# Tomeu7/AO-MARL

Hardware: AMD Instinct MI355X
Metric: env steps/sec (AO frames/sec) (higher is better)
Workload: dtype f32

## Files before the change

### __graft_entry__.py

```python
import os
import subprocess
import sys

ROOT = os.path.dirname(os.path.abspath(__file__))
if ROOT not in sys.path:
    sys.path.insert(0, ROOT)


def build():
    subprocess.check_call(["make", "-s", "-C", os.path.join(ROOT, "ao_marl_amd", "csrc")])
    subprocess.check_call(["make", "-s", "-C", os.path.join(ROOT, "oracle")])
    import ao_marl_amd
    from ao_marl_amd import libaomarl
    libaomarl.load()
    from oracle import aoref
    aoref.lib()


def smoke():
    import numpy as np
    import torch
    from ao_marl_amd.sim import HipSim
    from oracle import aoref
    sys.path.insert(0, os.path.join(ROOT, "tests"))
    from tests import helpers
    assert torch.cuda.is_available(), "smoke() needs a GPU"
    _, s, cal = helpers.calibrated("production_sh_10x10_2m")
    seeds = [1234, 1250]
    sim = HipSim(s, nenv=len(seeds))
    sim.set_modal(cal.volts2modes, cal.modes2volts)
    sim.reset(seeds)
    oracles = [aoref.OracleSim(s, seed=sd) for sd in seeds]
    for _ in range(2):
        sim.next_part_two(None)
        sim.next_part_one()
        for o in oracles:
            o.next_part_two(None)
            o.next_part_one()
    torch.cuda.synchronize()
    sl = sim.slopes.cpu().numpy()
    cm = sim.com.cpu().numpy()
    st = sim.strehl.cpu().numpy()
    for e, o in enumerate(oracles):
# ... 12 lines not shown
```

### ao_marl_amd/csrc/aomarl_capi.hip

```cpp
#include "aomarl_kernels.hip"

#include <math.h>
#include <stdlib.h>
#include <stdarg.h>
#include <stdio.h>
#include <string.h>

#include <algorithm>
#include <climits>
#include <string>
#include <vector>

static thread_local char g_err[512] = "";

int fail(const char *fmt, ...) {
  va_list ap;
  va_start(ap, fmt);
  vsnprintf(g_err, sizeof(g_err), fmt, ap);
  va_end(ap);
  return 1;
}


struct aomarl_ctx {
// ... 732 lines not shown
static Work work_layout(const aomarl_ctx *c, int nenv) {
  Work w;
  const DevSys &s = c->sys;
  const size_t ncol = (size_t)nenv * (c->nlayers > 0 ? c->nlayers : 1);
  w.ldz = (c->maxK + 3) & ~3;
  w.ldn = (c->maxdim + 3) & ~3;
  w.ldm = (s.nactu + 3) & ~3;
  const int W = 2 * s.hw, RB = 256 / W;
  w.nblk = (s.pupdiam + RB - 1) / RB;
  size_t o = 0;
  auto take = [&](size_t n) { size_t r = o; o += (n + 3) & ~(size_t)3; return r; };
  w.Z = take(ncol * w.ldz);
  w.NEWL = take(ncol * w.ldn);
  w.ZREF = take(ncol);
  w.Z2 = take(ncol * w.ldz);
  w.ZREF2 = take(ncol);
  w.MODES = take((size_t)nenv * w.ldm);
  w.TR = take((size_t)nenv * s.pupdiam * W * 2);
  w.TPART = take((size_t)nenv * w.nblk * 4);
  w.PEND = take((size_t)nenv * (W * W + 4));
  {
    size_t mn = std::max(ncol * (size_t)w.ldn, (size_t)nenv * (size_t)w.ldm);
    w.gemm_floats = 8 * mn;
    w.GEMM = take(w.gemm_floats);
    w.GEMM_ATM = take(w.gemm_floats);
  }
  w.total = o;
  return w;
}

size_t aomarl_workspace_floats(const aomarl_ctx *c, int nenv) {
  return c ? work_layout(c, nenv).total : 0;
}
size_t aomarl_screen_stride(const aomarl_ctx *c) { return c ? (size_t)c->sys.screen_stride : 0; }
size_t aomarl_dmshape_stride(const aomarl_ctx *c) { return c ? (size_t)c->sys.shape_stride : 0; }

static int check_range(const aomarl_ctx *c, const aomarl_state *st, int b, int n) {
  if (!c || !st) return fail("null ctx/state");
  if (c->pipe.active && !c->pipe_internal && st->screens == c->pipe.owner_screens)
    return fail("a pipelined frame is in flight on this state (aomarl_set_frame_pipeline): only aomarl_env_step and a "
                "full-range aomarl_reset are accepted until the reset -- slopes / voltage of odd frames are in the twin, "
                "the screens a frame ahead");
  if (b < 0 || n < 0 || b + n > st->nenv) return fail("env range [%d, %d) outside [0, %d)", b, b + n, st->nenv);
  if (st->ld_actu < c->sys.nactu) return fail("ld_actu (%d) < nactu (%d)", st->ld_actu, c->sys.nactu);
  if (!st->screens || !st->origin || !st->seeds || !st->ext_count || !st->com || !st->com1 ||
      !st->com2 || !st->err || !st->voltage || !st->slopes || !st->dm_shape || !st->strehl ||
      !st->le_img || !st->frame || !st->work)
    return fail("aomarl_state has a null mandatory buffer");
  return 0;
}

static DevState dev_state(const aomarl_state *st) {
  DevState d;
  d.nenv = st->nenv; d.ld_actu = st->ld_actu;
  d.screens = st->screens; d.origin = st->origin; d.seeds = st->seeds; d.ext_count = st->ext_count;
  d.com = st->com; d.com1 = st->com1; d.com2 = st->com2; d.err = st->err; d.voltage = st->voltage;
  d.slopes = st->slopes; d.dm_shape = st->dm_shape; d.bincube = st->bincube;
  d.wfs_phase = st->wfs_phase; d.tar_phase = st->tar_phase; d.strehl = st->strehl;
  d.le_img = st->le_img; d.frame = st->frame; d.work = st->work;
  d.origin_snap = nullptr;
  return d;
}

#include "aomarl_capi_atmos.hip"
#include "aomarl_capi_stages.hip"
#include "aomarl_capi_agents.hip"
// ... 4 lines not shown
```

### ao_marl_amd/csrc/aomarl_capi_composites.hip

```cpp
const char *aomarl_frame_kernel_name(aomarl_ctx *c) {
  if (!c || !c->fw_variant[0]) return "";
  snprintf(c->fw_name, sizeof(c->fw_name), "k_frame_wave<%d, %d, %s, %s, %s, %s>", c->fw_variant[0], c->fw_variant[1],
           c->fw_variant[2] ? "true" : "false", c->fw_variant[3] ? "true" : "false",
           c->fw_variant[4] ? "true" : "false", c->fw_variant[5] ? "true" : "false");
  return c->fw_name;
}

int aomarl_frame_kernel_time(aomarl_ctx *c, double *total_ms, int *launches) {
  if (!c || !total_ms || !launches) return fail("frame_kernel_time: null argument");
  double tot = 0.0;
  int n = 0;
  for (size_t i = 0; i + 1 < c->fw_ev_used; i += 2) {
    float ms = 0.f;
    HIPCHK(hipEventSynchronize(c->fw_ev[i + 1]));
    HIPCHK(hipEventElapsedTime(&ms, c->fw_ev[i], c->fw_ev[i + 1]));
    tot += ms; n++;
  }
  { const int rrc = fw_ev_rewind(c); if (rrc) return rrc; }
  *total_ms = tot; *launches = n;
  return 0;
}

int aomarl_frame_fused_available(aomarl_ctx *c) {
  return c && c->sys.fused_ok && !c->force_unfused_frame ? 1 : 0;
}

static int frame_fused_impl(aomarl_ctx *c, aomarl_state *st, int b, int n, int flags, void *stream, int slot);

int aomarl_frame_fused(aomarl_ctx *c, aomarl_state *st, int b, int n, int flags, void *stream) {
  return frame_fused_impl(c, st, b, n, flags, stream, -1);
}

static int frame_fused_impl(aomarl_ctx *c, aomarl_state *st, int b, int n, int flags, void *stream, int slot) {
  int rc = check_range(c, st, b, n);
  if (rc) return rc;
  if (slot < 0) {
    rc = atmos_wait_pending(c, stream);
    if (rc) return rc;
    rc = psf_wait_pending(c, stream);
    if (rc) return rc;
  }
  if (!c->sys.fused_ok) return fail("frame_fused: geometry not eligible (see aomarl_frame_fused_available)");
  if (flags & (AOMARL_IMG_FROM_PHASE_BUFFER | AOMARL_IMG_NO_ATMOS | AOMARL_IMG_NO_DMS))
    return fail("frame_fused: FROM_PHASE_BUFFER / NO_ATMOS / NO_DMS are not supported here");
  const bool noise = (flags & AOMARL_IMG_NOISE) && c->sys.noise >= 0.f;
  const bool cube = flags & AOMARL_IMG_WRITE_BINCUBE;
  const bool otf = flags & AOMARL_IMG_DM_FROM_VOLTAGE;
  const int cog = ((flags & AOMARL_IMG_COG) ? 1 : 0) | (c->fused_debug << 8);
  if (otf && !c->sys.otf_ok) return fail("frame_fused: DM_FROM_VOLTAGE needs a separable stack-array lattice (see aomarl_dm_from_voltage_available)");
  if (cube && !st->bincube) return fail("frame_fused: WRITE_BINCUBE needs st->bincube");
  if (!cube && !(cog & 1)) return fail("frame_fused: nothing to produce (neither bincube nor slopes)");
  if (n == 0) return 0;
  hipStream_t s = (hipStream_t)stream;
  Work w = work_layout(c, st->nenv);
  const int W = 2 * c->sys.hw;
  float *TR = st->work + w.TR + (size_t)b * c->sys.pupdiam * W * 2;
  float *TP = st->work + w.TPART + (size_t)b * w.nblk * 4;
  float *PEND = st->work + w.PEND + (size_t)b * (W * W + 4);
  DevState ds = dev_state(st);
  if (w.nblk != c->sys.ntiles) return fail("frame_fused: internal stripe count mismatch");
  const int nb = otf ? c->sys.otf_nb : 1;
  const bool hp = c->dft_mode < 0 ? g_precision != 0 : c->dft_mode == 1;
  const bool qf = FW_QF && otf && !hp && !noise && !cube;
  const bool dma = FW_DMA && otf && (hp || FW_DMA_F32);
  const size_t smm = sizeof(float) * ((qf ? 0 : 2 * 128) + (otf ? 4 * 4 * nb * c->sys.otf_latw : 0)) + FW_SLOT_BYTES(dma) +
                     (dma ? 4 * FWD_WAVE(c->nlayers == 1 ? 1 : 3) : 128) +
                     (qf ? 4 * 16 * (size_t)c->sys.ntiles : 0);
  static const long lds_pad_env = [] { const char *e = getenv("AOMARL_FW_LDS_PAD"); return e ? atol(e) : -1L; }();
  size_t lds_pad = 0;
  if (qf && slot >= 0 && smm >= 40 * 1024) {
    const size_t two_per_cu = (160 * 1024) / 3 + 64;
    lds_pad = lds_pad_env >= 0 ? (size_t)lds_pad_env : (smm < two_per_cu ? (two_per_cu - smm + 63) / 64 * 64 : 0);
    if (smm + lds_pad > 64 * 1024) lds_pad = 0;
  }
  dim3 grid((n + 3) / 4, c->sys.ntiles), blk(256);
#define FW(NL, NB, OTF, NZ, WC, HP) hipExtLaunchKernelGGL((k_frame_wave<NL, NB, OTF, NZ, WC, HP>), grid, blk, smm + lds_pad, s, ev_start, ev_done, 0, c->sys, ds, b, n, cog, TR, TP, w.nblk)
#define FW_H(NL, NB, OTF, NZ, WC) do { if (hp) FW(NL, NB, OTF, NZ, WC, true); else FW(NL, NB, OTF, NZ, WC, false); } while (0)
#define FW_NC(NL, NB, OTF)                                                                     \
  do {                                                                                          \
    if (noise) { if (cube) FW_H(NL, NB, OTF, true, true); else FW_H(NL, NB, OTF, true, false); }     \
    else { if (cube) FW_H(NL, NB, OTF, false, true); else FW_H(NL, NB, OTF, false, false); }         \
  } while (0)
#define FW_L(NL)                                                          \
  do {                                                                    \
    if (!otf) FW_NC(NL, 1, false);                                        \
    else if (nb == 1) FW_NC(NL, 1, true);                                 \
    else FW_NC(NL, 2, true);                                              \
  } while (0)
  const bool timed = !c->capturing && c->time_fw && c->fw_ev_used + 2 <= c->fw_ev.size();
  hipEvent_t ev_start = nullptr, ev_done = nullptr;
  if (c->prefetch_atmos) {
    rc = side_stream(c);
    if (rc) return rc;
    ev_done = slot < 0 ? c->ev_frame : c->pipe.ev_done[slot];
  }
  if (timed) { ev_start = c->fw_ev[c->fw_ev_used]; ev_done = c->fw_ev[c->fw_ev_used + 1]; c->fw_ev_used += 2; }
  hipEvent_t ev_mark = nullptr;
  if (c->capturing) { ev_mark = ev_done; ev_start = nullptr; ev_done = nullptr; }
  if (c->nlayers == 1) FW_L(1); else FW_L(3);
  if (ev_mark) { HIPCHK(hipEventRecord(ev_mark, s)); ev_done = ev_mark; }
  c->frame_marked = false;
  c->fw_variant[0] = c->nlayers == 1 ? 1 : 3; c->fw_variant[1] = otf ? nb : 1; c->fw_variant[2] = otf;
  c->fw_variant[3] = noise; c->fw_variant[4] = cube; c->fw_variant[5] = hp;
  g_arith[hp ? AR_FRAME_SPLIT : AR_FRAME_F32]++;
#undef FW_L
#undef FW_NC
#undef FW_H
// ... 189 lines not shown
```

### ao_marl_amd/csrc/aomarl_kernels.hip

```cpp
#include "aomarl_host.h"
#include "aomarl_gemm_p.h"
#include <type_traits>

#define WAVE 64

typedef unsigned u32x4 __attribute__((ext_vector_type(4)));

__device__ __forceinline__ hx2 cvt_h2(float a, float b) {
  return __builtin_bit_cast(hx2, __builtin_amdgcn_cvt_pkrtz(a, b));
}
__device__ __forceinline__ float sub_lo(hx2 h, float a) {
  float r;
  asm("v_fma_mix_f32 %0, %1, -1.0, %2 op_sel_hi:[1,0,0]" : "=v"(r) : "v"(h), "v"(a));
  return r;
}
__device__ __forceinline__ float sub_hi(hx2 h, float a) {
  float r;
  asm("v_fma_mix_f32 %0, %1, -1.0, %2 op_sel:[1,0,0] op_sel_hi:[1,0,0]" : "=v"(r) : "v"(h), "v"(a));
  return r;
}

struct __attribute__((packed, aligned(4))) f4u { float v[4]; };
__device__ __forceinline__ void add4(float acc[4], const float *p) {
  const f4u t = *reinterpret_cast<const f4u *>(p);
// ... 2056 lines not shown

typedef const int __attribute__((address_space(4))) *const_int_p;
typedef const float __attribute__((address_space(4))) *const_float_p;

template <int NL, bool OTF>
struct FrameRaw {
  float L[NL][4];
  float P[OTF ? 1 : 4], T[8];
  unsigned mrow;
  float F;
  f4u SH;
  float4 CS;
};

template <int NL, int NB, bool OTF, bool NOISE, bool WRITE_CUBE, bool HP>
#ifndef FW_WAVES
#define FW_WAVES 3
#endif
#ifndef FW_QF
#define FW_QF 1
#endif
#ifndef FW_DMA
#define FW_DMA 1
#endif
#ifndef FW_DEPTH
#define FW_DEPTH 2
#endif
#ifndef FW_DMA_F32
#define FW_DMA_F32 1
#endif
#ifndef FW_SLOTS1
#define FW_SLOTS1 0
#endif
#define FW_SLOT_BYTES(dma) ((dma) ? (FW_SLOTS1 ? 2 * 3 * 1024 : 16384) : 16384)
#define FWD_BLK 1152
#define FWD_IMG (2 * 1024 + 128)
#define FWD_WAVE(nl) ((nl) * FWD_IMG)
__global__ __launch_bounds__(256) __attribute__((amdgpu_waves_per_eu(FW_WAVES, FW_WAVES)))
void k_frame_wave(DevSys sys, DevState st, int env_begin,
                                                    int env_count, int do_cog,
                                                    float *__restrict__ TR,
                                                    float *__restrict__ TPART, int nblk) {
  extern __shared__ float smem[];
  const int pd = sys.pupdiam, ntl = sys.ntiles;
  const int tid = threadIdx.x, lane = tid & 63, q = lane >> 4, c = lane & 15;
  const int wv = __builtin_amdgcn_readfirstlane(tid >> 6);
  constexpr bool QF = FW_QF && OTF && !HP && !NOISE && !WRITE_CUBE;
  constexpr bool DMA = FW_DMA && OTF && (HP || FW_DMA_F32);
  float2 *sTw = reinterpret_cast<float2 *>(smem);
  float *lat_all = reinterpret_cast<float *>(sTw + (QF ? 0 : 128));
  float4 *shb = reinterpret_cast<float4 *>(lat_all + 4 * 4 * NB * (OTF ? sys.otf_latw : 0));
  char *dimg = reinterpret_cast<char *>(shb) + FW_SLOT_BYTES(DMA) + (DMA ? wv * FWD_WAVE(NL) : 0);
  float4 *qmom = reinterpret_cast<float4 *>(reinterpret_cast<char *>(shb) + FW_SLOT_BYTES(DMA) + (DMA ? 4 * FWD_WAVE(NL) : 0)) + wv * ntl;
  const int dbg = do_cog >> 8;
  do_cog &= 1;
  const int r = sys.stripe_order[blockIdx.y];
  const int el = 4 * blockIdx.x + wv;
  if constexpr (!QF) {
    if (tid < 128) {
      float sn, cs;
      sincospif((float)tid * (1.0f / 64.0f), &sn, &cs);
      sTw[tid] = make_float2(cs, sn);
    }
    __syncthreads();
  }
  const bool active = el < env_count;
  const int e = env_begin + (active ? el : env_count - 1);
// ... 130 lines not shown
  };

  auto tile = [&](int info, int infon, FrameRaw<NL, OTF> &cur, FrameRaw<NL, OTF> &nxt, auto mode_tag, float4 *dma_slot) {
    constexpr bool DM = decltype(mode_tag)::value == 1;
    constexpr bool NOFETCH = decltype(mode_tag)::value != 0;
    const int t = (info >> 24) & 0x7F;
    f32x4 S = PK ? NP4 : Z4;
    if (OTF) {
      f32x4 U = Z4;
#pragma unroll
      for (int kb = 0; kb < NB; kb++) {
        const float a = latq[(q + 4 * kb) * latw + t * tpn];
        U = mfma16(jm_ok ? a : 0.f, Pyr[kb], U);
      }
#pragma unroll
      for (int s = 0; s < NB; s++) S = mfma16(Pxr[s], U[s], S);
    }
    const float flux_i = cur.F;
    float4 *slot = DM ? dma_slot : shb + (nlit & 1) * 256;
    if constexpr (!DM) {
      nlit++;
      slot[wv * 64 + lane] = make_float4(cur.SH.v[0], cur.SH.v[1], cur.SH.v[2], cur.SH.v[3]);
#ifndef FW_DBG_NOBAR
      __syncthreads();
#endif
    }
    if (!(DM && FW_SLOTS1)) {
      const float4 t0 = slot[lane], t1 = slot[64 + lane];
      cur.T[0] = t0.x; cur.T[1] = t0.y; cur.T[2] = t0.z; cur.T[3] = t0.w;
      cur.T[4] = t1.x; cur.T[5] = t1.y; cur.T[6] = t1.z; cur.T[7] = t1.w;
      cur.CS = slot[128 + lane];
    }
    const float4 csP = cur.CS;
    float wr[4], wi[4], ar[4], ai[4];
    if constexpr (PK) {
      const f32x2 X01 = {cur.T[0], cur.T[1]}, X23 = {cur.T[2], cur.T[3]};
      const f32x2 Y01 = {cur.T[4], cur.T[5]}, Y23 = {cur.T[6], cur.T[7]};
      PK_GUARD_MFMA();
      f32x2 p01 = pk_fma_s(X01, c0c0, pk_lo(S)), p23 = pk_fma_s(X23, c0c0, pk_hi(S));
      p01 = pk_fma_s(Y01, c1c1, p01); p23 = pk_fma_s(Y23, c1c1, p23);
#pragma unroll
      for (int l = 0; l < NL; l++) {
        const f32x2 l01 = {cur.L[l][0], cur.L[l][1]}, l23 = {cur.L[l][2], cur.L[l][3]};
        p01 = pk_add(p01, l01); p23 = pk_add(p23, l23);
      }
      if (info & FW_FULL) {
        const f32x2 t01 = pk_mul_s(p01, wil2), t23 = pk_mul_s(p23, wil2);
        const f32x2 b01 = pk_mul_s(p01, til2), b23 = pk_mul_s(p23, til2);
        if constexpr (QF) {
          sdp += p01; sd2p = __builtin_elementwise_fma(p01, p01, sd2p);
          sdp += p23; sd2p = __builtin_elementwise_fma(p23, p23, sd2p);
          wr[0] = __builtin_amdgcn_cosf(t01.x); wi[0] = __builtin_amdgcn_sinf(t01.x);
          wr[1] = __builtin_amdgcn_cosf(t01.y); wi[1] = __builtin_amdgcn_sinf(t01.y);
          wr[2] = __builtin_amdgcn_cosf(t23.x); wi[2] = __builtin_amdgcn_sinf(t23.x);
          wr[3] = __builtin_amdgcn_cosf(t23.y); wi[3] = __builtin_amdgcn_sinf(t23.y);
        } else {
        sdp += p01; sd2p = __builtin_elementwise_fma(p01, p01, sd2p);
        const f32x2 r01 = {rintf(t01.x), rintf(t01.y)}, r23 = {rintf(t23.x), rintf(t23.y)};
        sdp += p23; sd2p = __builtin_elementwise_fma(p23, p23, sd2p);
        const f32x2 a01 = pk_fma_nc_s(p01, wil2, r01), a23 = pk_fma_nc_s(p23, wil2, r23);
        wr[0] = __builtin_amdgcn_cosf(a01.x); wi[0] = __builtin_amdgcn_sinf(a01.x);
        wr[1] = __builtin_amdgcn_cosf(a01.y); wi[1] = __builtin_amdgcn_sinf(a01.y);
        wr[2] = __builtin_amdgcn_cosf(a23.x); wi[2] = __builtin_amdgcn_sinf(a23.x);
        wr[3] = __builtin_amdgcn_cosf(a23.y); wi[3] = __builtin_amdgcn_sinf(a23.y);
        }
        ar[0] = __builtin_amdgcn_cosf(b01.x); ai[0] = __builtin_amdgcn_sinf(b01.x);
        ar[1] = __builtin_amdgcn_cosf(b01.y); ai[1] = __builtin_amdgcn_sinf(b01.y);
        ar[2] = __builtin_amdgcn_cosf(b23.x); ai[2] = __builtin_amdgcn_sinf(b23.x);
        ar[3] = __builtin_amdgcn_cosf(b23.y); ai[3] = __builtin_amdgcn_sinf(b23.y);
        nfull++;
      } else {
        const float ph4[4] = {p01.x, p01.y, p23.x, p23.y};
#pragma unroll
        for (int j = 0; j < 4; j++) {
          const float ph = ph4[j];
          const bool m = (cur.mrow >> (4 * q + j)) & 1u;
          float a_ = ph * wfs_il; a_ -= rintf(a_);
          const float b_ = sci_rev(ph, tar_il);
          wr[j] = m ? __builtin_amdgcn_cosf(a_) : 0.f; wi[j] = m ? __builtin_amdgcn_sinf(a_) : 0.f;
          ar[j] = m ? __builtin_amdgcn_cosf(b_) : 0.f; ai[j] = m ? __builtin_amdgcn_sinf(b_) : 0.f;
          const float d = m ? ph : 0.f;
          sd += d; sd2 += d * d; sm += m ? 1.f : 0.f;
        }
      }
    } else if (info & FW_FULL) {
#pragma unroll
      for (int j = 0; j < 4; j++) {
        float ph = (OTF ? S[j] : cur.P[OTF ? 0 : j]) + (c0 * cur.T[j] + c1 * cur.T[4 + j]);
#pragma unroll
        for (int l = 0; l < NL; l++) ph += cur.L[l][j];
        float a_ = ph * wfs_il; a_ -= rintf(a_);
        const float b_ = sci_rev(ph, tar_il);
        wr[j] = __builtin_amdgcn_cosf(a_); wi[j] = __builtin_amdgcn_sinf(a_);
        ar[j] = __builtin_amdgcn_cosf(b_); ai[j] = __builtin_amdgcn_sinf(b_);
        const float d = ph - pivot;
        sd += d; sd2 += d * d;
      }
      sm += 4.f;
    } else {
#pragma unroll
      for (int j = 0; j < 4; j++) {
        float ph = (OTF ? S[j] : cur.P[OTF ? 0 : j]) + (c0 * cur.T[j] + c1 * cur.T[4 + j]);
#pragma unroll
        for (int l = 0; l < NL; l++) ph += cur.L[l][j];
        const bool m = (cur.mrow >> (4 * q + j)) & 1u;
        float a_ = ph * wfs_il; a_ -= rintf(a_);
        const float b_ = sci_rev(ph, tar_il);
        wr[j] = m ? __builtin_amdgcn_cosf(a_) : 0.f; wi[j] = m ? __builtin_amdgcn_sinf(a_) : 0.f;
        ar[j] = m ? __builtin_amdgcn_cosf(b_) : 0.f; ai[j] = m ? __builtin_amdgcn_sinf(b_) : 0.f;
        const float d = m ? ph - pivot : 0.f;
        sd += d; sd2 += d * d; sm += m ? 1.f : 0.f;
      }
    }
    if constexpr (!NOFETCH) fetch(infon, nxt);
    if (!(dbg & 2)) {
      if constexpr (PK) {
        const f32x2 ar01 = {ar[0], ar[1]}, ar23 = {ar[2], ar[3]}, ai01 = {ai[0], ai[1]}, ai23 = {ai[2], ai[3]};
        PK_GUARD_TRANS();
        const f32x2 sr_ = pk_add(ar01, ar23), si_ = pk_add(ai01, ai23);
        pk_acc_add(R0rp, sr_); pk_acc_add(R0ip, si_);
        PK_END_TO_MFMA();
      } else {
        R0r += (ar[0] + ar[1]) + (ar[2] + ar[3]);
        R0i += (ai[0] + ai[1]) + (ai[2] + ai[3]);
      }
      if (HP) {
        const hx8 csH = __builtin_bit_cast(hx8, csP);
        hx8 arH, arL, aiH, aiL;
        dup_hl(ar[0], ar[1], ar[2], ar[3], arH, arL);
        dup_hl(ai[0], ai[1], ai[2], ai[3], aiH, aiL);
        PA = mfma_h(arH, csH, PA); PA = mfma_h(arL, csH, PA);
        PB = mfma_h(aiH, csH, PB); PB = mfma_h(aiL, csH, PB);
      } else {
        PA = mfma16(ar[0], csP.x, PA); PB = mfma16(ai[0], csP.x, PB);
        PA = mfma16(ar[1], csP.y, PA); PB = mfma16(ai[1], csP.y, PB);
        PA = mfma16(ar[2], csP.z, PA); PB = mfma16(ai[2], csP.z, PB);
        PA = mfma16(ar[3], csP.w, PA); PB = mfma16(ai[3], csP.w, PB);
      }
// ... 7 lines not shown
        if constexpr (QF) {
          const float z = spot_qf_moments(qfk, wr, wi, Z4);
          if (c == 0 && q < 3) reinterpret_cast<float *>(qmom + t)[q] = z;
        } else if constexpr (PK) spot_cog_f32_pk(sys, st, e, info & 0xFFFF, lane, Cc, Ss, wr, wi, do_cog, Z4);
        else spot_cog_f32(sys, st, e, info & 0xFFFF, lane, Cc, Ss, wr, wi, do_cog, Z4);
      } else {
        spot_core<NOISE, WRITE_CUBE>(sys, st, e, info & 0xFFFF, lane, Cc, Ss, wr, wi, do_cog, flux_i, Z4);
      }
    }
  };

  if constexpr (DMA) {
    const std::integral_constant<int, 1> dm;
    const int np = sys.pair_count[r];
    const const_int_p pinfo = (const_int_p)(unsigned long long)(sys.pair_info + r * (2 * ((ntl + 1) / 2 + 2)));
    const int rr = lane >> 3, kk = (lane & 7) ^ rr;
    unsigned dvo[NL][2];
#pragma unroll
    for (int l = 0; l < NL; l++) {
      const DevLayer &L = sys.layers[l];
      int py = L.toy + st.origin[(e * sys.nlayers + l) * 2 + 1]; py -= (py >= L.dim) ? L.dim : 0;
#pragma unroll
      for (int b = 0; b < 2; b++) {
        unsigned pr = (unsigned)(16 * r + 8 * b + rr) + (unsigned)py; pr = min(pr, pr - ldim[l]);
        dvo[l][b] = 4u * (pr * (ldim[l] + RING_PAD)) + 16u * (unsigned)kk;
      }
    }
    const int bc = c >> 3, rc = c & 7;
    const char *rdp[2];
#pragma unroll
    for (int h = 0; h < 2; h++) rdp[h] = dimg + bc * FWD_BLK + 16 * (rc * 8 + ((4 * h + q) ^ rc));
    const unsigned dimg_lds = (unsigned)(unsigned long long)dimg;
    FrameRaw<NL, OTF> A, B;
    unsigned mrA, mrB;
    float fA, fB;
    const unsigned shb_lds = (unsigned)(unsigned long long)shb + 1024u * (unsigned)wv;
    auto dma16 = [&](unsigned vo, __amdgpu_buffer_rsrc_t rs, unsigned lds_addr, unsigned so) {
      unsigned keep;
      asm volatile("s_mov_b32 %0, m0\n\ts_mov_b32 m0, %3\n\ts_nop 0\n\tbuffer_load_dwordx4 %1, %2, %4 offen lds\n\ts_mov_b32 m0, %0"
                   : "=&s"(keep) : "v"(vo), "s"(rs), "s"(lds_addr), "s"(so) : "memory");
    };
    auto issue_shared = [&](int ia, int ib, int par) {
      const int ta = (ia >> 24) & 0x7F, tb = (ib >> 24) & 0x7F;
      if (FW_SLOTS1) {
        if (wv < 3) {
          dma16(shvo, shrs, shb_lds, (unsigned)ta << shstep);
          dma16(shvo, shrs, shb_lds + 3072u, (unsigned)tb << shstep);
        }
      } else {
        dma16(shvo, shrs, shb_lds + (unsigned)par * 8192u, (unsigned)ta << shstep);
        dma16(shvo, shrs, shb_lds + (unsigned)par * 8192u + 4096u, (unsigned)tb << shstep);
      }
    };
    auto issue = [&](int ia, int ib) {
      const int ta = (ia >> 24) & 0x7F, tb = (ib >> 24) & 0x7F;
      mrA = *reinterpret_cast<const uint16_t *>(mkb + 2u * (unsigned)ta + mvo);
      mrB = *reinterpret_cast<const uint16_t *>(mkb + 2u * (unsigned)tb + mvo);
      fA = cflux[ia & 0xFFFF];
      fB = cflux[ib & 0xFFFF];
#pragma unroll
      for (int l = 0; l < NL; l++) {
        unsigned sx = 16u * (unsigned)(ta & ~1) + lpxs[l]; sx -= (sx >= ldim[l]) ? ldim[l] : 0u;
        const unsigned so = 4u * sx;
#pragma unroll
        for (int b = 0; b < 2; b++) dma16(dvo[l][b], lrs[l], dimg_lds + l * FWD_IMG + b * FWD_BLK, so);
      }
    };
    int ia = pinfo[0], ib = pinfo[1];
    if (np > 0) { issue_shared(ia, ib, 0); issue(ia, ib); }
    for (int k = 0; k < np; k++) {
      const int ja = pinfo[2 * k + 2], jb = pinfo[2 * k + 3];
      asm volatile("s_waitcnt vmcnt(0)" ::: "memory");
#pragma unroll
      for (int l = 0; l < NL; l++) {
        const float4 va = *reinterpret_cast<const float4 *>(rdp[0] + l * FWD_IMG);
        const float4 vb = *reinterpret_cast<const float4 *>(rdp[1] + l * FWD_IMG);
        A.L[l][0] = va.x; A.L[l][1] = va.y; A.L[l][2] = va.z; A.L[l][3] = va.w;
        B.L[l][0] = vb.x; B.L[l][1] = vb.y; B.L[l][2] = vb.z; B.L[l][3] = vb.w;
      }
      A.mrow = mrA; A.F = fA; B.mrow = mrB; B.F = fB;
      asm volatile("s_waitcnt lgkmcnt(0)" ::: "memory");
      if (FW_SLOTS1) {
        if (k + 1 < np) issue(ja, jb);
        __syncthreads();
        float4 *slots = shb;
        {
          const float4 a0 = slots[lane], a1 = slots[64 + lane];
          A.CS = slots[128 + lane];
          A.T[0] = a0.x; A.T[1] = a0.y; A.T[2] = a0.z; A.T[3] = a0.w; A.T[4] = a1.x; A.T[5] = a1.y; A.T[6] = a1.z; A.T[7] = a1.w;
        }
        if (ia & FW_LIT) tile(ia, 0, A, A, dm, slots);
        {
          const float4 b0 = slots[192 + lane], b1 = slots[256 + lane];
          B.CS = slots[320 + lane];
          B.T[0] = b0.x; B.T[1] = b0.y; B.T[2] = b0.z; B.T[3] = b0.w; B.T[4] = b1.x; B.T[5] = b1.y; B.T[6] = b1.z; B.T[7] = b1.w;
        }
        asm volatile("s_waitcnt lgkmcnt(0)" ::: "memory");
        __syncthreads();
        if (k + 1 < np) issue_shared(ja, jb, 0);
        if (ib & FW_LIT) tile(ib, 0, B, B, dm, slots);
      } else {
        float4 *slots = shb + (k & 1) * 512;
        __syncthreads();
        if (k + 1 < np) { issue_shared(ja, jb, (k + 1) & 1); issue(ja, jb); }
        if (ia & FW_LIT) tile(ia, 0, A, A, dm, slots);
        if (ib & FW_LIT) tile(ib, 0, B, B, dm, slots + 256);
      }
      ia = ja; ib = jb;
    }
  } else {
  const std::integral_constant<int, 0> nd;
  const std::integral_constant<int, 2> nf;
  const int nl = sys.lit_count[r];
  const const_int_p linfo = (const_int_p)(unsigned long long)(sys.lit_info + r * (ntl + 8));
  {
    constexpr int D = FW_DEPTH;
    FrameRaw<NL, OTF> raw[D];
    int inf[D];
#pragma unroll
    for (int d = 0; d < D; d++) { inf[d] = linfo[d]; fetch(inf[d], raw[d]); }
    const int rem = nl % D, nfull = nl - rem;
    for (int k = 0; k < nfull; k += D) {
      int nx[D];
#pragma unroll
      for (int d = 0; d < D; d++) nx[d] = linfo[k + D + d];
#pragma unroll
      for (int d = 0; d < D; d++) tile(inf[d], nx[d], raw[d], raw[d], nd, nullptr);
#pragma unroll
      for (int d = 0; d < D; d++) inf[d] = nx[d];
    }
#pragma unroll
    for (int d = 0; d + 1 < D; d++)
      if (rem > d) tile(inf[d], inf[d], raw[d], raw[d], nf, nullptr);
  }
  }
  if (!active) return;
  if constexpr (QF) {
    if (do_cog && !(dbg & 1)) {
      for (int tt = lane; tt < ntl; tt += 64) {
// ... 830 lines not shown
```

### ao_marl_amd/libaomarl.py

```python
import ctypes as C
import os
import subprocess

import numpy as np

HERE = os.path.dirname(os.path.abspath(__file__))
LIB_PATH = os.environ.get("AOMARL_LIB") or os.path.join(HERE, "libaomarl_hip.so")
MAX_LAYERS, MAX_DMS, ABI_VERSION = 8, 4, 2
PRECISION_F32, PRECISION_SPLIT_F16 = 0, 1

DM_PZT, DM_TT = 0, 1
TRACE_ATMOS, TRACE_DMS, TRACE_RESET, TRACE_MASK = 1, 2, 4, 8
IMG_FROM_PHASE_BUFFER, IMG_NOISE, IMG_WRITE_BINCUBE, IMG_COG, IMG_NO_ATMOS, IMG_NO_DMS = \
    1, 2, 4, 8, 16, 32
IMG_DM_FROM_VOLTAGE = 64
APPLY_COMP_VOLTAGE, APPLY_DEFER_STACK_SHAPE = 1, 2

_fp = C.POINTER(C.c_float)
_ip = C.POINTER(C.c_int32)
_up = C.POINTER(C.c_uint32)


class DmDesc(C.Structure):
    _fields_ = [("type", C.c_int32), ("dim", C.c_int32), ("nact", C.c_int32),
# ... 107 lines not shown
    ("aomarl_actor_forward", _i, [_vp, _vp, _vp, C.c_uint32, C.c_uint32, _vp, _vp, _vp]),
    ("aomarl_env_step", _i, [_vp, C.POINTER(State), _vp, _vp, _f, _fp, _fp, _vp, _vp, _vp]),
    ("aomarl_policy_env_step", _i, [_vp, C.POINTER(State), _vp, _vp, _vp, _vp, C.c_uint32, C.c_uint32, _f, _fp, _fp,
                                    _vp, _vp, _vp, _vp, _vp]),
    ("aomarl_env_step_shortcut", _i, [_vp, _vp]),
    ("aomarl_do_control_reduced", _i, [_vp, C.POINTER(State), _vp]),
    ("aomarl_graph_stats", _i, [_vp, C.POINTER(C.c_ulonglong), C.POINTER(C.c_ulonglong)]),
    ("aomarl_set_frame_pipeline", _i, [_vp, C.POINTER(State), C.POINTER(State)]),
    ("aomarl_frame_pipeline_state", _i, [_vp, C.POINTER(_i), C.POINTER(_i), C.POINTER(C.c_ulonglong),
                                         C.POINTER(C.c_ulonglong)]),
    ("aomarl_frame_kernel_name", C.c_char_p, [_vp]),
    ("aomarl_frame_kernel_time", _i, [_vp, C.POINTER(C.c_double), C.POINTER(_i)]),
    ("aomarl_denoiser_create", _i, [C.POINTER(_fp), C.POINTER(_fp), C.POINTER(C.c_void_p)]),
    ("aomarl_denoiser_apply", _i, [_vp, _vp, C.c_longlong, _vp]),
    ("aomarl_denoiser_apply_f32", _i, [_vp, _vp, C.c_longlong, _vp]),
    ("aomarl_denoiser_apply_split_f16", _i, [_vp, _vp, C.c_longlong, _vp]),
    ("aomarl_denoiser_overflow", _i, [_vp, C.POINTER(C.c_uint), _vp]),
    ("aomarl_denoiser_destroy", _i, [_vp]),
    ("aomarl_denoiser_trainer_create", _i, [C.POINTER(_fp), C.POINTER(_fp), C.c_double, C.c_double, C.c_double,
                                            C.c_double, _i, C.POINTER(C.c_void_p)]),
    ("aomarl_denoiser_trainer_destroy", _i, [_vp]),
    ("aomarl_denoiser_trainer_step", _i, [_vp, _vp, _vp, C.c_longlong, _vp, _vp]),
    ("aomarl_denoiser_trainer_grads", _i, [_vp, _vp, _vp, C.c_longlong, C.POINTER(C.c_void_p),
                                           C.POINTER(C.c_void_p), _vp, _vp]),
    ("aomarl_denoiser_trainer_get", _i, [_vp, C.POINTER(C.c_void_p), C.POINTER(C.c_void_p), _vp]),
    ("aomarl_target_psf_buffer", _i, _range + [_vp]),
    ("aomarl_set_geo", _i, [_vp, _fp]),
    ("aomarl_geo_workspace_floats", C.c_size_t, [_vp, _i]),
    ("aomarl_geo_control", _i, _range + [_vp, _vp]),
    ("aomarl_frame_fused_available", _i, [_vp]),
    ("aomarl_dm_from_voltage_available", _i, [_vp]),
    ("aomarl_materialize_dm_shape", _i, _range + [_vp]),
    ("aomarl_frame_fused", _i, _range + [_i, _vp]),
    ("aomarl_comp_strehl", _i, _range + [_vp]),
    ("aomarl_reset_strehl", _i, _range + [_vp]),
    ("aomarl_volts2modes", _i, [_vp, C.POINTER(State), _i, _vp, _i, _vp, _vp]),
    ("aomarl_set_slopes2modes", _i, [_vp, _i, _fp]),
    ("aomarl_slopes2modes", _i, _range + [_vp, _vp]),
    ("aomarl_next_part_one", _i, _range + [_fp, _fp, _i, _vp]),
    ("aomarl_next_part_two", _i, _range + [_vp, _vp]),
    ("aomarl_gemm_nt", _i, [_i, _i, _i, _f, _vp, _i, _vp, _i, _f, _vp, _i, _vp]),
    ("aomarl_gemm_nt_split", _i, [_i, _i, _i, _f, _vp, _i, _vp, _i, _f, _vp, _i, _f, _f, _vp, C.c_longlong, _vp]),
    ("aomarl_gemm_nt_batched", _i, [_i, _i, _i, _i, _vp, _i, C.c_longlong, _vp, _i, C.c_longlong,
                                    _vp, C.c_longlong, _vp, _i, C.c_longlong, _i, _vp]),
]

_lib = None


class SacDesc(C.Structure):
    _fields_ = [(n, C.c_int32) for n in ("n_agents", "batch", "in_max", "act_max", "hidden", "hidden_critic",
                                         "n_hidden",
                                         "state_dim", "action_dim")] + \
               [("state_gather", C.c_void_p), ("action_gather", C.c_void_p), ("n_act", C.c_void_p),
                ("target_entropy", C.c_void_p)] + \
               [(n, C.c_float) for n in ("gamma", "tau", "lr", "beta1", "beta2", "adam_eps", "log_sig_min",
                                         "log_sig_max", "action_scale", "action_bias")] + \
               [(n, C.c_void_p) for n in ("policy", "policy_m", "policy_v", "policy_grad", "critic",
                                          "critic_m", "critic_v", "critic_grad", "critic_target",
                                          "log_alpha", "log_alpha_m", "log_alpha_v", "log_alpha_grad",
                                          "alpha")]


class ActorDesc(C.Structure):
    _fields_ = [(n, C.c_int32) for n in ("n_agents", "nenv", "state_dim", "in_max", "act_max", "hidden",
                                         "n_hidden", "action_dim")] + \
# ... 306 lines not shown
```

### include/aomarl.h

```cpp
#ifndef AOMARL_H
#define AOMARL_H
#include <stddef.h>
#include <stdint.h>

#ifdef __cplusplus
extern "C" {
#endif

#define AOMARL_MAX_LAYERS 8
#define AOMARL_MAX_DMS 4
#define AOMARL_ABI_VERSION 2

enum { AOMARL_DM_PZT = 0, AOMARL_DM_TT = 1 };

enum { AOMARL_TRACE_ATMOS = 1, AOMARL_TRACE_DMS = 2, AOMARL_TRACE_RESET = 4,
       AOMARL_TRACE_MASK = 8  };
enum {
  AOMARL_IMG_FROM_PHASE_BUFFER = 1,
  AOMARL_IMG_NOISE = 2,
  AOMARL_IMG_WRITE_BINCUBE = 4,
  AOMARL_IMG_COG = 8,
  AOMARL_IMG_NO_ATMOS = 16,
  AOMARL_IMG_NO_DMS = 32,
  AOMARL_IMG_DM_FROM_VOLTAGE = 64
// ... 127 lines not shown
                           int flags, void *stream);
int aomarl_comp_image(aomarl_ctx *ctx, aomarl_state *st, int env_begin, int env_count, int flags,
                      void *stream);
int aomarl_do_centroids(aomarl_ctx *ctx, aomarl_state *st, int env_begin, int env_count,
                        void *stream);
int aomarl_slopes_geom(aomarl_ctx *ctx, aomarl_state *st, int env_begin, int env_count,
                       void *stream);
int aomarl_do_control(aomarl_ctx *ctx, aomarl_state *st, int env_begin, int env_count,
                      void *stream);
int aomarl_set_com(aomarl_ctx *ctx, aomarl_state *st, int env_begin, int env_count,
                   const float *com_dev, void *stream);
int aomarl_rl_control(aomarl_ctx *ctx, aomarl_state *st, int env_begin, int env_count,
                      const float *action_dev, void *stream);
int aomarl_rl_control_modes(aomarl_ctx *ctx, aomarl_state *st, int env_begin, int env_count,
                            const float *m0_dev, const float *m1_dev, float g,
                            const float *action_dev, float *modes_out_dev, void *stream);
int aomarl_apply_control(aomarl_ctx *ctx, aomarl_state *st, int env_begin, int env_count,
                         int comp_voltage, void *stream);
int aomarl_dm_from_voltage_available(aomarl_ctx *ctx);
int aomarl_materialize_dm_shape(aomarl_ctx *ctx, aomarl_state *st, int env_begin, int env_count,
                                void *stream);
int aomarl_comp_dm_shape(aomarl_ctx *ctx, aomarl_state *st, int env_begin, int env_count,
                         const float *volts_dev, void *stream);
int aomarl_get_dm_shape(aomarl_ctx *ctx, aomarl_state *st, int env_begin, int env_count, int k,
                        float *dst, void *stream);
int aomarl_set_option(aomarl_ctx *ctx, const char *name, int value);
int aomarl_target_psf(aomarl_ctx *ctx, aomarl_state *st, int env_begin, int env_count,
                      void *stream);
int aomarl_frame_fused_available(aomarl_ctx *ctx);
const char *aomarl_frame_kernel_name(aomarl_ctx *ctx);
int aomarl_frame_kernel_time(aomarl_ctx *ctx, double *total_ms, int *launches);
int aomarl_frame_fused(aomarl_ctx *ctx, aomarl_state *st, int env_begin, int env_count, int flags,
                       void *stream);
int aomarl_gemm_batched(int batch, int transA, int transB, int M, int N, int K, const float *A, int lda,
                        long long strideA, const float *B, int ldb, long long strideB, const float *bias,
                        long long strideBias, float *C, int ldc, long long strideC, int relu,
                        int accumulate, void *stream);
typedef struct {
  int32_t n_agents, batch, in_max, act_max, hidden, hidden_critic, n_hidden;
  int32_t state_dim, action_dim;
  const int32_t *state_gather;
  const int32_t *action_gather;
  const int32_t *n_act;
  const float *target_entropy;
  float gamma, tau, lr, beta1, beta2, adam_eps;
  float log_sig_min, log_sig_max, action_scale, action_bias;
  float *policy, *policy_m, *policy_v, *policy_grad;
  float *critic, *critic_m, *critic_v, *critic_grad, *critic_target;
  float *log_alpha, *log_alpha_m, *log_alpha_v, *log_alpha_grad, *alpha;
} aomarl_sac_desc;
typedef struct aomarl_sac aomarl_sac;
#define AOMARL_SAC_SOFT_UPDATE 1
#define AOMARL_SAC_TUNE_ALPHA 2
int aomarl_sac_layout(const aomarl_sac_desc *d, long long *policy_off, long long *critic_off,
                      long long *policy_len, long long *critic_len);
int aomarl_sac_create(const aomarl_sac_desc *d, aomarl_sac **out);
int aomarl_sac_destroy(aomarl_sac *s);
int aomarl_sac_update(aomarl_sac *s, const float *state, const float *next_state, const float *action,
                      const float *reward, const float *mask, long long replay_rows, const int64_t *idx,
                      const float *eps_next, const float *eps_pi, uint32_t seed, uint32_t counter,
                      int adam_step, int flags, float *losses, void *stream);
int aomarl_split_states(int nenv, int state_dim, int n_agents, int in_max, const int32_t *gather,
                        const float *state, float *out, void *stream);
int aomarl_policy_sample(int nenv, int act_max, int action_dim, const float *head, float log_sig_min,
                         float log_sig_max, float scale, float bias, const int32_t *sc_agent,
                         const int32_t *sc_local, const float *eps, uint32_t seed, uint32_t counter,
// ... 117 lines not shown
```

Baseline: 553,800.

## Shrink fused-frame LDS slots, load masks lazily and skip unused flux loads

Shrinks the DMA shared-screen slot buffer from four to three quarter-slots so only three waves stage data, which lowers the fused frame kernel's LDS request. It also defers the pupil-mask row load to the point of use and skips per-tile flux loads when noise and cube output are off. The LDS padding rule now pads whenever three blocks plus an assumed product-kernel reservation would not fit in a CU, replacing the old fixed threshold. New C API queries for LDS bytes and work layout are added, and the build now fetches kernel variants in parallel. The risk is that the smaller slots and lazy loads add latency inside the tile loop or change occupancy in unexpected ways.

```diff
diff --git a/__graft_entry__.py b/__graft_entry__.py
--- a/__graft_entry__.py
+++ b/__graft_entry__.py
@@ -8,7 +8,14 @@
 
 
 def build():
-    subprocess.check_call(["make", "-s", "-C", os.path.join(ROOT, "ao_marl_amd", "csrc")])
+    csrc = os.path.join(ROOT, "ao_marl_amd", "csrc")
+    variant = subprocess.Popen(["make", "-s", "-C", csrc, "fw_fetch_all"])
+    try:
+        subprocess.check_call(["make", "-s", "-C", csrc])
+    finally:
+        rc = variant.wait()
+    if rc:
+        raise subprocess.CalledProcessError(rc, "make fw_fetch_all")
     subprocess.check_call(["make", "-s", "-C", os.path.join(ROOT, "oracle")])
     import ao_marl_amd
     from ao_marl_amd import libaomarl
diff --git a/ao_marl_amd/csrc/aomarl_capi.hip b/ao_marl_amd/csrc/aomarl_capi.hip
--- a/ao_marl_amd/csrc/aomarl_capi.hip
+++ b/ao_marl_amd/csrc/aomarl_capi.hip
@@ -788,6 +788,15 @@
 size_t aomarl_workspace_floats(const aomarl_ctx *c, int nenv) {
   return c ? work_layout(c, nenv).total : 0;
 }
+int aomarl_frame_work_layout(const aomarl_ctx *c, int nenv, size_t *offset, size_t *floats) {
+  if (!c || nenv < 1 || !offset || !floats) return fail("frame_work_layout: bad argument");
+  const Work w = work_layout(c, nenv);
+  const size_t W = 2 * (size_t)c->sys.hw;
+  offset[0] = w.TR; floats[0] = (size_t)nenv * c->sys.pupdiam * W * 2;
+  offset[1] = w.TPART; floats[1] = (size_t)nenv * w.nblk * 4;
+  offset[2] = w.PEND; floats[2] = (size_t)nenv * (W * W + 4);
+  return 0;
+}
 size_t aomarl_screen_stride(const aomarl_ctx *c) { return c ? (size_t)c->sys.screen_stride : 0; }
 size_t aomarl_dmshape_stride(const aomarl_ctx *c) { return c ? (size_t)c->sys.shape_stride : 0; }
 
diff --git a/ao_marl_amd/csrc/aomarl_capi_composites.hip b/ao_marl_amd/csrc/aomarl_capi_composites.hip
--- a/ao_marl_amd/csrc/aomarl_capi_composites.hip
+++ b/ao_marl_amd/csrc/aomarl_capi_composites.hip
@@ -29,6 +29,35 @@
 
 int aomarl_frame_fused(aomarl_ctx *c, aomarl_state *st, int b, int n, int flags, void *stream) {
   return frame_fused_impl(c, st, b, n, flags, stream, -1);
+}
+
+static size_t fw_lds_request(int nlayers, int nb, int latw, int ntiles, bool otf, bool noise, bool cube, bool hp) {
+  const bool qf = FW_QF && otf && !hp && !noise && !cube;
+  const bool dma = FW_DMA && otf && (hp || FW_DMA_F32);
+  return sizeof(float) * ((qf ? 0 : 2 * 128) + (otf ? 4 * 4 * nb * latw : 0)) + FW_SLOT_BYTES(dma) +
+         (dma ? 4 * FWD_WAVE(nlayers == 1 ? 1 : 3) : 128) + (qf ? 4 * 16 * (size_t)ntiles : 0);
+}
+
+static const size_t FW_CU_LDS = 160 * 1024, FW_PRODUCT_LDS = 46080;
+static size_t fw_lds_pad(size_t smm) {
+  static const long lds_pad_env = [] { const char *e = getenv("AOMARL_FW_LDS_PAD"); return e ? atol(e) : -1L; }();
+  if (3 * smm + FW_PRODUCT_LDS <= FW_CU_LDS) return 0;
+  const size_t two_per_cu = FW_CU_LDS / 3 + 64;
+  size_t lds_pad = lds_pad_env >= 0 ? (size_t)lds_pad_env : (smm < two_per_cu ? (two_per_cu - smm + 63) / 64 * 64 : 0);
+  if (smm + lds_pad > 64 * 1024) lds_pad = 0;
+  return lds_pad;
+}
+
+int aomarl_frame_lds_bytes(int nlayers, int lattice_blocks, int lattice_width, int ntiles, int image_flags, int split_f16,
+                           int pipelined, size_t *request, size_t *launch) {
+  if (nlayers < 1 || lattice_blocks < 1 || lattice_blocks > 2 || lattice_width < 0 || ntiles < 1 || !request || !launch)
+    return fail("frame_lds_bytes: bad argument");
+  const bool otf = image_flags & AOMARL_IMG_DM_FROM_VOLTAGE, noise = image_flags & AOMARL_IMG_NOISE;
+  const bool cube = image_flags & AOMARL_IMG_WRITE_BINCUBE, hp = split_f16 != 0;
+  const bool qf = FW_QF && otf && !hp && !noise && !cube;
+  *request = fw_lds_request(nlayers, otf ? lattice_blocks : 1, lattice_width, ntiles, otf, noise, cube, hp);
+  *launch = *request + (qf && pipelined ? fw_lds_pad(*request) : 0);
+  return 0;
 }
 
 static int frame_fused_impl(aomarl_ctx *c, aomarl_state *st, int b, int n, int flags, void *stream, int slot) {
@@ -62,17 +91,8 @@
   const int nb = otf ? c->sys.otf_nb : 1;
   const bool hp = c->dft_mode < 0 ? g_precision != 0 : c->dft_mode == 1;
   const bool qf = FW_QF && otf && !hp && !noise && !cube;
-  const bool dma = FW_DMA && otf && (hp || FW_DMA_F32);
-  const size_t smm = sizeof(float) * ((qf ? 0 : 2 * 128) + (otf ? 4 * 4 * nb * c->sys.otf_latw : 0)) + FW_SLOT_BYTES(dma) +
-                     (dma ? 4 * FWD_WAVE(c->nlayers == 1 ? 1 : 3) : 128) +
-                     (qf ? 4 * 16 * (size_t)c->sys.ntiles : 0);
-  static const long lds_pad_env = [] { const char *e = getenv("AOMARL_FW_LDS_PAD"); return e ? atol(e) : -1L; }();
-  size_t lds_pad = 0;
-  if (qf && slot >= 0 && smm >= 40 * 1024) {
-    const size_t two_per_cu = (160 * 1024) / 3 + 64;
-    lds_pad = lds_pad_env >= 0 ? (size_t)lds_pad_env : (smm < two_per_cu ? (two_per_cu - smm + 63) / 64 * 64 : 0);
-    if (smm + lds_pad > 64 * 1024) lds_pad = 0;
-  }
+  const size_t smm = fw_lds_request(c->nlayers, nb, c->sys.otf_latw, c->sys.ntiles, otf, noise, cube, hp);
+  const size_t lds_pad = qf && slot >= 0 ? fw_lds_pad(smm) : 0;
   dim3 grid((n + 3) / 4, c->sys.ntiles), blk(256);
 #define FW(NL, NB, OTF, NZ, WC, HP) hipExtLaunchKernelGGL((k_frame_wave<NL, NB, OTF, NZ, WC, HP>), grid, blk, smm + lds_pad, s, ev_start, ev_done, 0, c->sys, ds, b, n, cog, TR, TP, w.nblk)
 #define FW_H(NL, NB, OTF, NZ, WC) do { if (hp) FW(NL, NB, OTF, NZ, WC, true); else FW(NL, NB, OTF, NZ, WC, false); } while (0)
diff --git a/ao_marl_amd/csrc/aomarl_kernels.hip b/ao_marl_amd/csrc/aomarl_kernels.hip
--- a/ao_marl_amd/csrc/aomarl_kernels.hip
+++ b/ao_marl_amd/csrc/aomarl_kernels.hip
@@ -2112,7 +2112,17 @@
 #ifndef FW_SLOTS1
 #define FW_SLOTS1 0
 #endif
-#define FW_SLOT_BYTES(dma) ((dma) ? (FW_SLOTS1 ? 2 * 3 * 1024 : 16384) : 16384)
+#ifndef FW_SH3
+#define FW_SH3 1
+#endif
+#ifndef FW_MASK_LAZY
+#define FW_MASK_LAZY 1
+#endif
+#ifndef FW_FLUX_CX
+#define FW_FLUX_CX 1
+#endif
+#define FW_SHQ (FW_SH3 ? 3 : 4)
+#define FW_SLOT_BYTES(dma) ((dma) ? (FW_SLOTS1 ? 2 * 3 * 1024 : 2 * 2 * FW_SHQ * 1024) : 16384)
 #define FWD_BLK 1152
 #define FWD_IMG (2 * 1024 + 128)
 #define FWD_WAVE(nl) ((nl) * FWD_IMG)
@@ -2309,6 +2319,10 @@
       cur.CS = slot[128 + lane];
     }
     const float4 csP = cur.CS;
+    auto mask_row = [&](const FrameRaw<NL, OTF> &raw) -> unsigned {
+      if constexpr (DM && FW_MASK_LAZY) return *reinterpret_cast<const uint16_t *>(mkb + 2u * (unsigned)t + mvo);
+      else return raw.mrow;
+    };
     float wr[4], wi[4], ar[4], ai[4];
     if constexpr (PK) {
       const f32x2 X01 = {cur.T[0], cur.T[1]}, X23 = {cur.T[2], cur.T[3]};
@@ -2348,10 +2362,11 @@
         nfull++;
       } else {
         const float ph4[4] = {p01.x, p01.y, p23.x, p23.y};
+        const unsigned mrow = mask_row(cur);
 #pragma unroll
         for (int j = 0; j < 4; j++) {
           const float ph = ph4[j];
-          const bool m = (cur.mrow >> (4 * q + j)) & 1u;
+          const bool m = (mrow >> (4 * q + j)) & 1u;
           float a_ = ph * wfs_il; a_ -= rintf(a_);
           const float b_ = sci_rev(ph, tar_il);
           wr[j] = m ? __builtin_amdgcn_cosf(a_) : 0.f; wi[j] = m ? __builtin_amdgcn_sinf(a_) : 0.f;
@@ -2375,12 +2390,13 @@
       }
       sm += 4.f;
     } else {
+      const unsigned mrow = mask_row(cur);
 #pragma unroll
       for (int j = 0; j < 4; j++) {
         float ph = (OTF ? S[j] : cur.P[OTF ? 0 : j]) + (c0 * cur.T[j] + c1 * cur.T[4 + j]);
 #pragma unroll
         for (int l = 0; l < NL; l++) ph += cur.L[l][j];
-        const bool m = (cur.mrow >> (4 * q + j)) & 1u;
+        const bool m = (mrow >> (4 * q + j)) & 1u;
         float a_ = ph * wfs_il; a_ -= rintf(a_);
         const float b_ = sci_rev(ph, tar_il);
         wr[j] = m ? __builtin_amdgcn_cosf(a_) : 0.f; wi[j] = m ? __builtin_amdgcn_sinf(a_) : 0.f;
@@ -2454,8 +2470,8 @@
     for (int h = 0; h < 2; h++) rdp[h] = dimg + bc * FWD_BLK + 16 * (rc * 8 + ((4 * h + q) ^ rc));
     const unsigned dimg_lds = (unsigned)(unsigned long long)dimg;
     FrameRaw<NL, OTF> A, B;
-    unsigned mrA, mrB;
-    float fA, fB;
+    unsigned mrA = 0, mrB = 0;
+    float fA = 0.f, fB = 0.f;
     const unsigned shb_lds = (unsigned)(unsigned long long)shb + 1024u * (unsigned)wv;
     auto dma16 = [&](unsigned vo, __amdgpu_buffer_rsrc_t rs, unsigned lds_addr, unsigned so) {
       unsigned keep;
@@ -2469,17 +2485,21 @@
           dma16(shvo, shrs, shb_lds, (unsigned)ta << shstep);
           dma16(shvo, shrs, shb_lds + 3072u, (unsigned)tb << shstep);
         }
-      } else {
-        dma16(shvo, shrs, shb_lds + (unsigned)par * 8192u, (unsigned)ta << shstep);
-        dma16(shvo, shrs, shb_lds + (unsigned)par * 8192u + 4096u, (unsigned)tb << shstep);
+      } else if (!FW_SH3 || wv < 3) {
+        dma16(shvo, shrs, shb_lds + (unsigned)par * (2048u * FW_SHQ), (unsigned)ta << shstep);
+        dma16(shvo, shrs, shb_lds + (unsigned)par * (2048u * FW_SHQ) + 1024u * FW_SHQ, (unsigned)tb << shstep);
       }
     };
     auto issue = [&](int ia, int ib) {
       const int ta = (ia >> 24) & 0x7F, tb = (ib >> 24) & 0x7F;
-      mrA = *reinterpret_cast<const uint16_t *>(mkb + 2u * (unsigned)ta + mvo);
-      mrB = *reinterpret_cast<const uint16_t *>(mkb + 2u * (unsigned)tb + mvo);
-      fA = cflux[ia & 0xFFFF];
-      fB = cflux[ib & 0xFFFF];
+      if (!FW_MASK_LAZY) {
+        mrA = *reinterpret_cast<const uint16_t *>(mkb + 2u * (unsigned)ta + mvo);
+        mrB = *reinterpret_cast<const uint16_t *>(mkb + 2u * (unsigned)tb + mvo);
+      }
+      if constexpr (!FW_FLUX_CX || NOISE || WRITE_CUBE) {
+        fA = cflux[ia & 0xFFFF];
+        fB = cflux[ib & 0xFFFF];
+      }
 #pragma unroll
       for (int l = 0; l < NL; l++) {
         unsigned sx = 16u * (unsigned)(ta & ~1) + lpxs[l]; sx -= (sx >= ldim[l]) ? ldim[l] : 0u;
@@ -2522,11 +2542,11 @@
         if (k + 1 < np) issue_shared(ja, jb, 0);
         if (ib & FW_LIT) tile(ib, 0, B, B, dm, slots);
       } else {
-        float4 *slots = shb + (k & 1) * 512;
+        float4 *slots = shb + (k & 1) * (128 * FW_SHQ);
         __syncthreads();
         if (k + 1 < np) { issue_shared(ja, jb, (k + 1) & 1); issue(ja, jb); }
         if (ia & FW_LIT) tile(ia, 0, A, A, dm, slots);
-        if (ib & FW_LIT) tile(ib, 0, B, B, dm, slots + 256);
+        if (ib & FW_LIT) tile(ib, 0, B, B, dm, slots + 64 * FW_SHQ);
       }
       ia = ja; ib = jb;
     }
diff --git a/ao_marl_amd/libaomarl.py b/ao_marl_amd/libaomarl.py
--- a/ao_marl_amd/libaomarl.py
+++ b/ao_marl_amd/libaomarl.py
@@ -163,6 +163,8 @@
     ("aomarl_dm_from_voltage_available", _i, [_vp]),
     ("aomarl_materialize_dm_shape", _i, _range + [_vp]),
     ("aomarl_frame_fused", _i, _range + [_i, _vp]),
+    ("aomarl_frame_lds_bytes", _i, [_i, _i, _i, _i, _i, _i, _i, C.POINTER(C.c_size_t), C.POINTER(C.c_size_t)]),
+    ("aomarl_frame_work_layout", _i, [_vp, _i, C.POINTER(C.c_size_t), C.POINTER(C.c_size_t)]),
     ("aomarl_comp_strehl", _i, _range + [_vp]),
     ("aomarl_reset_strehl", _i, _range + [_vp]),
     ("aomarl_volts2modes", _i, [_vp, C.POINTER(State), _i, _vp, _i, _vp, _vp]),
diff --git a/include/aomarl.h b/include/aomarl.h
--- a/include/aomarl.h
+++ b/include/aomarl.h
@@ -183,6 +183,9 @@
 int aomarl_frame_kernel_time(aomarl_ctx *ctx, double *total_ms, int *launches);
 int aomarl_frame_fused(aomarl_ctx *ctx, aomarl_state *st, int env_begin, int env_count, int flags,
                        void *stream);
+int aomarl_frame_lds_bytes(int nlayers, int lattice_blocks, int lattice_width, int ntiles, int image_flags,
+                           int split_f16, int pipelined, size_t *request, size_t *launch);
+int aomarl_frame_work_layout(const aomarl_ctx *ctx, int nenv, size_t offset[3], size_t floats[3]);
 int aomarl_gemm_batched(int batch, int transA, int transB, int M, int N, int K, const float *A, int lda,
                         long long strideA, const float *B, int ldb, long long strideB, const float *bias,
                         long long strideBias, float *C, int ldc, long long strideC, int relu,
```

Result: no change. 558,200 (median of 6 runs) (+0.8%).
